# Aedelon/MASt3R-SLAM

Measured on AMD Instinct MI355X. Metric: keyframe-pairs/sec (512x512 two-view infer+match+GN), higher is better.
Workload: dtype fp16

## Files before the change

### mast3r-slam_amd/csrc/attention.hip

```cpp
#include "gemm_common.h"
#include <cstdlib>
#include <type_traits>

namespace {

using m3gemm::bf16x8;
using m3gemm::f32x4;
using m3gemm::bf16_t;
using m3gemm::glds16;
using m3gemm::pack16;
using m3gemm::mfma16;
using m3gemm::DT_BF16;
using m3gemm::DT_F16;
typedef __attribute__((ext_vector_type(4))) short bf16x4;
typedef float f32x2 __attribute__((ext_vector_type(2)));

constexpr int kThreads = 256;
constexpr int QROWS = 128;
constexpr int KT = 64;
constexpr int HD = 64;
constexpr int kTileBytes = KT * HD * 2;
constexpr int kLds = 4 * kTileBytes;

using m3gemm::pack_bf16;

struct AttnArgs {
    const bf16_t *Q, *K, *V;
    bf16_t *O;
    int q_row_stride, kv_row_stride, o_row_stride;
    long long q_batch_stride, kv_batch_stride, o_batch_stride;
    int Tq, Tk, heads, nbatch, kv_batch_shift;
    float scale_log2e;
};

#ifndef M3_ATTN_ABL
#define M3_ATTN_ABL 0
#endif
#ifndef M3_ATTN_EXP
#define M3_ATTN_EXP 0
#endif
constexpr float kDefer = 8.0f;
template <int QT, int DT, int MODE, int PVDT = DT>
__global__ void __launch_bounds__(kThreads, (MODE == 1 && QT == 2) ? 3 : 4)
k_attn(const AttnArgs a) {
    static_assert(MODE != 2 || PVDT == DT_BF16, "the deferred-maximum loop needs the fp32 exponent range of bf16 for P");
    constexpr int QR = QT * 64;
    __shared__ __attribute__((aligned(16))) unsigned char lds[kLds];
    const int tid = threadIdx.x, lane = tid & 63, wave = tid >> 6;
    const int lq = lane & 15, g = lane >> 4;
    const int nq = (a.Tq + QR - 1) / QR, nwg = gridDim.x;
    const int per = nwg >> 3, rem = nwg & 7, xcd = blockIdx.x & 7;
    const int id = (xcd < rem ? xcd * (per + 1) : rem * (per + 1) + (xcd - rem) * per) + (blockIdx.x >> 3);
    const int qblk = id % nq, head = (id / nq) % a.heads, b = id / (nq * a.heads);
    const int kvb = (b + a.kv_batch_shift) % a.nbatch;
    const bf16_t *Qp = a.Q + (size_t)b * a.q_batch_stride + head * HD;
    const bf16_t *Kp = a.K + (size_t)kvb * a.kv_batch_stride + head * HD;
    const bf16_t *Vp = a.V + (size_t)kvb * a.kv_batch_stride + head * HD;

    bf16x8 qf[QT][2];
#pragma unroll
    for (int qt = 0; qt < QT; ++qt) {
        int row = qblk * QR + wave * (16 * QT) + qt * 16 + lq;
        row = row < a.Tq ? row : a.Tq - 1;
#pragma unroll
        for (int ks = 0; ks < 2; ++ks)
            qf[qt][ks] = *reinterpret_cast<const bf16x8 *>(Qp + (size_t)row * a.q_row_stride + ks * 32 + g * 8);
    }

    const int srow = tid >> 3, sc = tid & 7;
    const int kch = sc ^ ((srow >> 1) & 7);
    const int vch = sc ^ (((srow >> 1) & 3) << 1);
    auto stage = [&](int t, int buf) {
        unsigned char *kb = lds + buf * 2 * kTileBytes, *vb = kb + kTileBytes;
#pragma unroll
        for (int i = 0; i < 2; ++i) {
            int kr = t * KT + i * 32 + srow;
            kr = kr < a.Tk ? kr : a.Tk - 1;
            const size_t row = (size_t)kr * a.kv_row_stride;
            glds16(Kp + row + kch * 8, kb + i * 4096 + wave * 1024);
            glds16(Vp + row + vch * 8, vb + i * 4096 + wave * 1024);
        }
    };

    f32x4 o[QT][4];
    float m_run[QT], l_run[QT];
    bool ovf = false;
    const int nt = (a.Tk + KT - 1) / KT;
    const int tq = lq >> 2, tp = lq & 3;

    auto run = [&](auto mode_tag) {
        constexpr int MD = decltype(mode_tag)::value;
        f32x4 l_acc[QT];
        bf16x8 ones;
#pragma unroll
        for (int j = 0; j < 8; ++j) ones[j] = (short)(PVDT == DT_BF16 ? 0x3F80 : 0x3C00);
#pragma unroll
        for (int qt = 0; qt < QT; ++qt) {
            m_run[qt] = -INFINITY; l_run[qt] = 0.f;
            l_acc[qt] = f32x4{0.f, 0.f, 0.f, 0.f};
#pragma unroll
            for (int dt = 0; dt < 4; ++dt) o[qt][dt] = f32x4{0.f, 0.f, 0.f, 0.f};
        }
        stage(0, 0);
        for (int t = 0; t < nt; ++t) {
            const int buf = t & 1;
            asm volatile("s_waitcnt vmcnt(0)" ::: "memory");
            m3gemm::lds_barrier();
            if (t + 1 < nt && !(M3_ATTN_ABL & 4)) stage(t + 1, buf ^ 1);
            const unsigned char *Ks = lds + ((M3_ATTN_ABL & 4) ? 0 : buf) * 2 * kTileBytes, *Vs = Ks + kTileBytes;

            if constexpr (MD == 2) {
                bool big = false;
#pragma unroll
                for (int qt = 0; qt < QT; ++qt) big |= l_acc[qt][0] > 0x1p60f;
                if (t > 0 && __any(big)) {
                    asm volatile("; rare path" ::: "memory");
#pragma unroll
                    for (int qt = 0; qt < QT; ++qt) {
                        const bool hit = l_acc[qt][0] > 0x1p60f;
                        ovf |= !(l_acc[qt][0] <= 0x1p100f);
                        const float alpha = hit ? 0x1p-64f : 1.0f;
                        m_run[qt] += hit ? 64.0f : 0.0f;
#pragma unroll
                        for (int r = 0; r < 4; ++r) l_acc[qt][r] *= alpha;
#pragma unroll
                        for (int dt = 0; dt < 4; ++dt)
#pragma unroll
                            for (int r = 0; r < 4; ++r) o[qt][dt][r] *= alpha;
                    }
                }
            }

            f32x4 s[QT][4];
#pragma unroll
            for (int qt = 0; qt < QT; ++qt) {
                const float c0 = (MD >= 1 && t > 0) ? -m_run[qt] : 0.f;
#pragma unroll
                for (int kt = 0; kt < 4; ++kt) s[qt][kt] = f32x4{c0, c0, c0, c0};
            }
#pragma unroll
            for (int ks = 0; ks < 2; ++ks)
#pragma unroll
                for (int kt = 0; kt < 4; ++kt) {
                    const int r = kt * 16 + lq;
                    const int c = (ks * 4 + g) ^ ((r >> 1) & 7);
                    bf16x8 kf;
                    if ((M3_ATTN_ABL & 1) && t > 0) { kf = qf[0][ks]; asm volatile("" : "+v"(kf)); }
                    else kf = *reinterpret_cast<const bf16x8 *>(Ks + r * 128 + c * 16);
#pragma unroll
                    for (int qt = 0; qt < QT; ++qt)
                        s[qt][kt] = mfma16<DT>(kf, qf[qt][ks], s[qt][kt]);
                }

            if (t == nt - 1 && (a.Tk & (KT - 1))) {
                const int kbase = t * KT + g * 4;
#pragma unroll
                for (int qt = 0; qt < QT; ++qt)
#pragma unroll
                    for (int kt = 0; kt < 4; ++kt)
#pragma unroll
                        for (int r = 0; r < 4; ++r)
                            if (kbase + kt * 16 + r >= a.Tk) s[qt][kt][r] = -INFINITY;
            }

            bf16x8 pf[QT][2];
            auto tile_max = [&](int qt) {
                float mx = fmaxf(__builtin_fmaxf(s[qt][0][0], s[qt][0][1]), s[qt][0][2]);
#pragma unroll
                for (int kt = 0; kt < 4; ++kt)
#pragma unroll
                    for (int r = (kt == 0 ? 3 : 0); r < 4; r += 2)
                        mx = (r + 1 < 4) ? fmaxf(__builtin_fmaxf(mx, s[qt][kt][r]), s[qt][kt][r + 1]) : fmaxf(mx, s[qt][kt][r]);
                mx = fmaxf(mx, __shfl_xor(mx, 16, 64));
                return fmaxf(mx, __shfl_xor(mx, 32, 64));
            };
            auto pack_p = [&](int qt) {
#pragma unroll
                for (int kk = 0; kk < 2; ++kk) {
                    union { unsigned u[4]; bf16x8 v; } pk;
                    pk.u[0] = pack16<PVDT>(s[qt][2 * kk][0], s[qt][2 * kk][1]);
                    pk.u[1] = pack16<PVDT>(s[qt][2 * kk][2], s[qt][2 * kk][3]);
                    pk.u[2] = pack16<PVDT>(s[qt][2 * kk + 1][0], s[qt][2 * kk + 1][1]);
                    pk.u[3] = pack16<PVDT>(s[qt][2 * kk + 1][2], s[qt][2 * kk + 1][3]);
                    pf[qt][kk] = pk.v;
                }
            };
            if constexpr (MD == 2) {
#pragma unroll
                for (int qt = 0; qt < QT; ++qt) {
                    if (t == 0) {
                        const float mx = tile_max(qt);
                        m_run[qt] = mx;
#pragma unroll
                        for (int kt = 0; kt < 4; ++kt)
#pragma unroll
                            for (int r = 0; r < 4; ++r) s[qt][kt][r] -= mx;
                    }
#pragma unroll
                    for (int kt = 0; kt < 4; ++kt)
#pragma unroll
                        for (int r = 0; r < 4; ++r) s[qt][kt][r] = (M3_ATTN_EXP >= 4) ? s[qt][kt][r] : __builtin_amdgcn_exp2f(s[qt][kt][r]);
#if M3_ATTN_EXP == 1
                    for (int kt = 0; kt < 4; ++kt) for (int r = 0; r < 4; ++r) l_run[qt] += s[qt][kt][r];
#endif
#if M3_ATTN_EXP == 5
                    pf[qt][0] = ones; pf[qt][1] = ones;
                    asm volatile("" :: "v"(s[qt][0]), "v"(s[qt][1]), "v"(s[qt][2]), "v"(s[qt][3]));
#else
                    pack_p(qt);
#endif
                }
            } else if constexpr (MD == 1) {
#pragma unroll
                for (int qt = 0; qt < QT; ++qt) {
                    const float mx = tile_max(qt);
                    if (t == 0) {
                        m_run[qt] = mx;
#pragma unroll
                        for (int kt = 0; kt < 4; ++kt)
#pragma unroll
                            for (int r = 0; r < 4; ++r) s[qt][kt][r] -= mx;
                    } else if (__any(mx > kDefer)) {
                        asm volatile("; rare path: keep it a branch (if-converted, its 32 subtracts + selects ran on every tile)" ::: "memory");
                        const float delta = fmaxf(mx, 0.f);
                        const float alpha = __builtin_amdgcn_exp2f(-delta);
                        m_run[qt] += delta;
                        l_run[qt] *= alpha;
#pragma unroll
                        for (int dt = 0; dt < 4; ++dt)
#pragma unroll
                            for (int r = 0; r < 4; ++r) o[qt][dt][r] *= alpha;
#pragma unroll
                        for (int kt = 0; kt < 4; ++kt)
#pragma unroll
                            for (int r = 0; r < 4; ++r) s[qt][kt][r] -= delta;
                    }
                    f32x2 rs2 = {0.f, 0.f};
#pragma unroll
                    for (int kt = 0; kt < 4; ++kt) {
#pragma unroll
                        for (int r = 0; r < 4; ++r) s[qt][kt][r] = __builtin_amdgcn_exp2f(s[qt][kt][r]);
                        rs2 += f32x2{s[qt][kt][0], s[qt][kt][1]};
                        rs2 += f32x2{s[qt][kt][2], s[qt][kt][3]};
                    }
                    l_run[qt] += rs2.x + rs2.y;
                    pack_p(qt);
                }
            } else {
#pragma unroll
                for (int qt = 0; qt < QT; ++qt) {
                    float mx = s[qt][0][0];
#pragma unroll
                    for (int kt = 0; kt < 4; ++kt)
#pragma unroll
                        for (int r = 0; r < 4; ++r) mx = fmaxf(mx, s[qt][kt][r]);
                    mx = fmaxf(mx, __shfl_xor(mx, 16, 64));
                    mx = fmaxf(mx, __shfl_xor(mx, 32, 64));
                    const float m_new = fmaxf(m_run[qt], mx);
                    const float alpha = __builtin_amdgcn_exp2f((m_run[qt] - m_new) * a.scale_log2e);
                    const float mb = m_new * a.scale_log2e;
                    m_run[qt] = m_new;
                    float rs = 0.f;
#pragma unroll
                    for (int kt = 0; kt < 4; ++kt)
#pragma unroll
                        for (int r = 0; r < 4; ++r) {
                            const float p = __builtin_amdgcn_exp2f(s[qt][kt][r] * a.scale_log2e - mb);
                            s[qt][kt][r] = p;
                            rs += p;
                        }
                    l_run[qt] = l_run[qt] * alpha + rs;
                    if (!__all(alpha == 1.0f)) {
#pragma unroll
                        for (int dt = 0; dt < 4; ++dt)
#pragma unroll
                            for (int r = 0; r < 4; ++r) o[qt][dt][r] *= alpha;
                    }
                    pack_p(qt);
                }
            }

#pragma unroll
            for (int kk = 0; kk < 2; ++kk) {
#pragma unroll
                for (int dt = 0; dt < 4; ++dt) {
                    union { bf16x4 h[2]; bf16x8 v; } vf;
                    if ((M3_ATTN_ABL & 2) && t > 0) { vf.v = qf[0][kk]; asm volatile("" : "+v"(vf.v)); }
                    else
#pragma unroll
                    for (int half = 0; half < 2; ++half) {
                        const int row = (2 * kk + half) * 16 + g * 4 + tq;
                        const int ch = (dt * 2 + (tp >> 1)) ^ (((row >> 1) & 3) << 1);
                        const unsigned char *p = Vs + row * 128 + ch * 16 + (tp & 1) * 8;
                        vf.h[half] = __builtin_amdgcn_ds_read_tr16_b64_v4i16(
                            (__attribute__((address_space(3))) bf16x4 *)p);
                    }
#pragma unroll
                    for (int qt = 0; qt < QT; ++qt)
                        o[qt][dt] = mfma16<PVDT>(vf.v, pf[qt][kk], o[qt][dt]);
                }
                if constexpr (MD == 2) {
#pragma unroll
                    for (int qt = 0; qt < QT; ++qt) l_acc[qt] = mfma16<PVDT>(ones, pf[qt][kk], l_acc[qt]);
                }
            }
        }
        m3gemm::lds_barrier();
        if constexpr (MD == 2 && M3_ATTN_EXP != 1) {
#pragma unroll
            for (int qt = 0; qt < QT; ++qt) l_run[qt] = l_acc[qt][0];
        } else {
#pragma unroll
            for (int qt = 0; qt < QT; ++qt) {
                float l = l_run[qt];
                l += __shfl_xor(l, 16, 64);
                l_run[qt] = l + __shfl_xor(l, 32, 64);
            }
        }
    };

    if constexpr (MODE == 2) {
        run(std::integral_constant<int, 2>{});
        bool bad = ovf;
#pragma unroll
        for (int qt = 0; qt < QT; ++qt) {
            bad |= !(l_run[qt] > 0.f && l_run[qt] <= 0x1p100f);
            float osum = 0.f;
#pragma unroll
            for (int dt = 0; dt < 4; ++dt) osum += (o[qt][dt][0] + o[qt][dt][1]) + (o[qt][dt][2] + o[qt][dt][3]);
            bad |= !(fabsf(osum) < INFINITY);
        }
#if M3_ATTN_EXP == 3
        bad = true;
#endif
        int *flag = reinterpret_cast<int *>(lds);
        if (tid == 0) *flag = 0;
        m3gemm::lds_barrier();
        if (__any(bad) && lane == 0) atomicOr(flag, 1);
        m3gemm::lds_barrier();
        const int redo = *reinterpret_cast<volatile int *>(flag);
        m3gemm::lds_barrier();
        if (redo) run(std::integral_constant<int, 1>{});
    } else {
        run(std::integral_constant<int, MODE>{});
    }

#pragma unroll
    for (int qt = 0; qt < QT; ++qt) {
        const float inv = 1.0f / l_run[qt];
        const int row = qblk * QR + wave * (16 * QT) + qt * 16 + lq;
        if (row >= a.Tq) continue;
        bf16_t *op = a.O + (size_t)b * a.o_batch_stride + (size_t)row * a.o_row_stride + head * HD;
#pragma unroll
        for (int dt = 0; dt < 4; ++dt) {
            uint2 w;
            w.x = pack16<DT>(o[qt][dt][0] * inv, o[qt][dt][1] * inv);
            w.y = pack16<DT>(o[qt][dt][2] * inv, o[qt][dt][3] * inv);
            *reinterpret_cast<uint2 *>(op + dt * 16 + g * 4) = w;
        }
    }
}

template <int DT>
__global__ void __launch_bounds__(kThreads)
k_rope2d(bf16_t *__restrict__ X, const int *__restrict__ pos_yx, const float *__restrict__ cs, int row_stride,
         int tokens, int heads, int tokens_per_image) {
    const int idx = blockIdx.x * kThreads + threadIdx.x;
    const int total = tokens * heads * 2;
    if (idx >= total) return;
    const int blk = idx & 1, head = (idx >> 1) % heads, tok = (idx >> 1) / heads;
    const int pos = pos_yx[(tok % tokens_per_image) * 2 + blk];
    bf16_t *p = X + (size_t)tok * row_stride + head * HD + blk * 32;
    union { uint4 q[4]; bf16_t h[32]; } v;
#pragma unroll
    for (int i = 0; i < 4; ++i) v.q[i] = reinterpret_cast<const uint4 *>(p)[i];
    const float *t = cs + (size_t)pos * 32;
#pragma unroll
    for (int i = 0; i < 16; ++i) {
        const float c = t[2 * i], sn = t[2 * i + 1];
        const float x1 = m3gemm::lo16<DT>(v.h[i]), x2 = m3gemm::lo16<DT>(v.h[i + 16]);
        const unsigned pk = pack16<DT>(x1 * c - x2 * sn, x2 * c + x1 * sn);
        v.h[i] = (bf16_t)(pk & 0xffff);
        v.h[i + 16] = (bf16_t)(pk >> 16);
    }
#pragma unroll
    for (int i = 0; i < 4; ++i) reinterpret_cast<uint4 *>(p)[i] = v.q[i];
}

}

extern "C" {

static int attention_launch(const void *Q, const void *K, const void *V, void *O, int q_row_stride, int kv_row_stride,
                            int o_row_stride, int64_t q_batch_stride, int64_t kv_batch_stride, int64_t o_batch_stride,
                            int nbatch, int heads, int Tq, int Tk, int kv_batch_shift, float scale, int dtype, bool pre,
                            void *stream) {
    M3_REQUIRE(Q && K && V && O && nbatch > 0 && heads > 0 && Tq > 0 && Tk > 0);
    M3_REQUIRE((dtype == DT_BF16 || dtype == DT_F16 || (dtype == 2 && pre)) && ((int64_t)Tq / 64 + 1) * heads * nbatch < (1ll << 31));
    M3_REQUIRE(q_row_stride % 8 == 0 && kv_row_stride % 8 == 0 && o_row_stride % 4 == 0);
    M3_REQUIRE(kv_batch_shift >= 0);
    AttnArgs a;
    a.Q = (const bf16_t *)Q; a.K = (const bf16_t *)K; a.V = (const bf16_t *)V; a.O = (bf16_t *)O;
    a.q_row_stride = q_row_stride; a.kv_row_stride = kv_row_stride; a.o_row_stride = o_row_stride;
    a.q_batch_stride = q_batch_stride; a.kv_batch_stride = kv_batch_stride; a.o_batch_stride = o_batch_stride;
    a.Tq = Tq; a.Tk = Tk; a.heads = heads; a.nbatch = nbatch; a.kv_batch_shift = kv_batch_shift;
    a.scale_log2e = scale * 1.4426950408889634f;
    const int64_t wg128 = (int64_t)m3_cdiv(Tq, QROWS) * heads * nbatch;
    const int64_t wg64 = (int64_t)m3_cdiv(Tq, 64) * heads * nbatch;
    hipStream_t st = (hipStream_t)stream;
    static const bool safe_bf16 = [] { const char *e = getenv("M3_ATTN_SAFE"); return e && atoi(e) != 0; }();
#define M3_ATTN(QTV, GRID)                                                                                  \
    do {                                                                                                    \
        if (dtype == 2) hipLaunchKernelGGL((k_attn<QTV, DT_F16, 2, DT_BF16>), dim3((unsigned)(GRID)), dim3(kThreads), 0, st, a); \
        else if (dtype == DT_F16) { if (pre) hipLaunchKernelGGL((k_attn<QTV, DT_F16, 1>), dim3((unsigned)(GRID)), dim3(kThreads), 0, st, a); \
                               else hipLaunchKernelGGL((k_attn<QTV, DT_F16, 0>), dim3((unsigned)(GRID)), dim3(kThreads), 0, st, a); } \
        else { if (pre) { if (safe_bf16) hipLaunchKernelGGL((k_attn<QTV, DT_BF16, 1>), dim3((unsigned)(GRID)), dim3(kThreads), 0, st, a); \
                          else hipLaunchKernelGGL((k_attn<QTV, DT_BF16, 2>), dim3((unsigned)(GRID)), dim3(kThreads), 0, st, a); }          \
               else hipLaunchKernelGGL((k_attn<QTV, DT_BF16, 0>), dim3((unsigned)(GRID)), dim3(kThreads), 0, st, a); }                    \
    } while (0)
    if (wg128 >= 512) M3_ATTN(2, wg128); else M3_ATTN(1, wg64);
#undef M3_ATTN
    M3_CHECK_LAUNCH("m3_attention");
    return M3_OK;
}

int m3_attention_dt(const void *Q, const void *K, const void *V, void *O, int q_row_stride, int kv_row_stride,
                    int o_row_stride, int64_t q_batch_stride, int64_t kv_batch_stride, int64_t o_batch_stride,
                    int nbatch, int heads, int Tq, int Tk, int kv_batch_shift, float scale, int dtype, void *stream) {
    return attention_launch(Q, K, V, O, q_row_stride, kv_row_stride, o_row_stride, q_batch_stride, kv_batch_stride,
                            o_batch_stride, nbatch, heads, Tq, Tk, kv_batch_shift, scale, dtype, false, stream);
}
int m3_attention_prescaled_dt(const void *Q, const void *K, const void *V, void *O, int q_row_stride, int kv_row_stride,
                              int o_row_stride, int64_t q_batch_stride, int64_t kv_batch_stride, int64_t o_batch_stride,
                              int nbatch, int heads, int Tq, int Tk, int kv_batch_shift, int dtype, void *stream) {
    return attention_launch(Q, K, V, O, q_row_stride, kv_row_stride, o_row_stride, q_batch_stride, kv_batch_stride,
                            o_batch_stride, nbatch, heads, Tq, Tk, kv_batch_shift, 1.0f, dtype, true, stream);
}
int m3_rope2d_dt(void *X, const int32_t *pos_yx, const float *cos_sin, int row_stride, int tokens, int heads,
                 int tokens_per_image, int dtype, void *stream) {
    M3_REQUIRE(X && pos_yx && cos_sin && tokens > 0 && heads > 0 && tokens_per_image > 0 && row_stride % 8 == 0);
    M3_REQUIRE(dtype == DT_BF16 || dtype == DT_F16);
    const int64_t total = (int64_t)tokens * heads * 2;
    if (dtype == DT_F16)
        hipLaunchKernelGGL(k_rope2d<DT_F16>, dim3(m3_cdiv(total, kThreads)), dim3(kThreads), 0, (hipStream_t)stream,
                           (bf16_t *)X, pos_yx, cos_sin, row_stride, tokens, heads, tokens_per_image);
    else
        hipLaunchKernelGGL(k_rope2d<DT_BF16>, dim3(m3_cdiv(total, kThreads)), dim3(kThreads), 0, (hipStream_t)stream,
                           (bf16_t *)X, pos_yx, cos_sin, row_stride, tokens, heads, tokens_per_image);
    M3_CHECK_LAUNCH("m3_rope2d");
    return M3_OK;
}

}
```

### mast3r-slam_amd/csrc/gemm_common.h

```cpp
#pragma once
#include "common.h"
#include "../../include/m3slam_model.h"

namespace m3gemm {

typedef __attribute__((ext_vector_type(8))) short bf16x8;
typedef __attribute__((ext_vector_type(4))) float f32x4;
typedef unsigned short bf16_t;

constexpr int BK = 64;

__device__ __forceinline__ float bf2f(bf16_t v) { return __uint_as_float((unsigned)v << 16); }
__device__ __forceinline__ bf16_t f2bf(float f) {
    unsigned u = __float_as_uint(f);
    if ((u & 0x7fffffffu) > 0x7f800000u) return (bf16_t)((u >> 16) | 0x40);
    return (bf16_t)((u + 0x7fffu + ((u >> 16) & 1u)) >> 16);
}
typedef float f32x2 __attribute__((ext_vector_type(2)));
__device__ __forceinline__ f32x2 gelu_erf2(f32x2 x) {
    f32x2 z = x * 0.70710678118654752f;
    z.x = __builtin_amdgcn_fmed3f(z.x, -3.0f, 3.0f);
    z.y = __builtin_amdgcn_fmed3f(z.y, -3.0f, 3.0f);
    const f32x2 u = z * z;
    f32x2 p = (f32x2)(4.074053805e-08f);
    p = __builtin_elementwise_fma(p, u, (f32x2)(-1.944763426e-06f));
    p = __builtin_elementwise_fma(p, u, (f32x2)(4.105960033e-05f));
    p = __builtin_elementwise_fma(p, u, (f32x2)(-5.110292695e-04f));
    p = __builtin_elementwise_fma(p, u, (f32x2)(4.235391971e-03f));
    p = __builtin_elementwise_fma(p, u, (f32x2)(-2.510276809e-02f));
    p = __builtin_elementwise_fma(p, u, (f32x2)(1.110792086e-01f));
    p = __builtin_elementwise_fma(p, u, (f32x2)(-3.753148019e-01f));
    p = __builtin_elementwise_fma(p, u, (f32x2)(1.128268361e+00f));
    const f32x2 hx = x * 0.5f;
    return __builtin_elementwise_fma(hx, z * p, hx);
}

typedef __bf16 m3_bf16x2 __attribute__((ext_vector_type(2)));
typedef _Float16 m3_f16x2 __attribute__((ext_vector_type(2)));
__device__ __forceinline__ unsigned pack_bf16(float lo, float hi) {
    return __builtin_bit_cast(unsigned, __builtin_convertvector(f32x2{lo, hi}, m3_bf16x2));
}

enum { DT_BF16 = 0, DT_F16 = 1 };
typedef __attribute__((ext_vector_type(8))) _Float16 f16x8;
template <int DT> __device__ __forceinline__ unsigned pack16(float lo, float hi) {
    if constexpr (DT == DT_BF16) return pack_bf16(lo, hi);
    else return __builtin_bit_cast(unsigned, __builtin_convertvector(f32x2{lo, hi}, m3_f16x2));
}
template <int DT> __device__ __forceinline__ float lo16(unsigned q) {
    if constexpr (DT == DT_BF16) return __uint_as_float(q << 16);
    else return (float)__builtin_bit_cast(_Float16, (unsigned short)(q & 0xffffu));
}
template <int DT> __device__ __forceinline__ float hi16(unsigned q) {
    if constexpr (DT == DT_BF16) return __uint_as_float(q & 0xffff0000u);
    else return (float)__builtin_bit_cast(_Float16, (unsigned short)(q >> 16));
}
template <int DT> __device__ __forceinline__ f32x4 mfma16(bf16x8 a, bf16x8 b, f32x4 c) {
    if constexpr (DT == DT_BF16) return __builtin_amdgcn_mfma_f32_16x16x32_bf16(a, b, c, 0, 0, 0);
    else return __builtin_amdgcn_mfma_f32_16x16x32_f16(__builtin_bit_cast(f16x8, a), __builtin_bit_cast(f16x8, b), c, 0, 0, 0);
}

typedef __attribute__((ext_vector_type(8))) short s16x8;
__device__ __forceinline__ bf16x8 relu_frag(bf16x8 v) {
    return __builtin_elementwise_max(v, (bf16x8)(short)0);
}

__device__ __forceinline__ void glds16(const void *g, void *lds_wave_base) {
    __builtin_amdgcn_global_load_lds((const __attribute__((address_space(1))) unsigned *)g,
                                     (__attribute__((address_space(3))) unsigned *)lds_wave_base, 16, 0, 0);
}

__device__ __forceinline__ void lds_barrier() {
    __builtin_amdgcn_sched_barrier(0);
    asm volatile("s_waitcnt lgkmcnt(0)" ::: "memory");
    __builtin_amdgcn_s_barrier();
    __builtin_amdgcn_sched_barrier(0);
}

struct GemmArgs {
    const bf16_t *A;
    const bf16_t *W;
    const float *bias;
    void *C;
    const void *R;
    const bf16_t *zero16;
    int M, N, K, ldc;
    int H, Wd, Cin, OH, OW, stride;
    const int *rope_pos;
    float rope_log2_base;
    int tokens_per_image, rope_cols;
    int ln_gsz, ln_tops;
    int rope_pmax;
    int q_cols;
    float q_scale;
    const bf16_t *W2;
    const float *bias2;
    long long a_gstride, c_gstride;
    int groups;
    int splits;
    int slices;
    float *C2;
    int dt;
    int relu_a;
    int v_bf16;
    void *C16;
    float *stats_out;
    int stats_w;
    const void *R_lo;
    void *C_lo;
    const float *ln_stats;
    const float *ln_colsum, *ln_colsum2;
    int ln_slots;
    float ln_eps;
    long long ln_gstride, stats_gstride;
};

template <int EPI>
__device__ __forceinline__ GemmArgs select_group(const GemmArgs &in, int grp) {
    GemmArgs g = in;
    if (grp == 1) {
        constexpr long long esz = (EPI == 2  || EPI == 3 ) ? 4 : 2;
        g.A = in.A + in.a_gstride;
        g.W = in.W2;
        g.bias = in.bias2;
        g.C = reinterpret_cast<unsigned char *>(in.C) + in.c_gstride * esz;
        if (in.R) g.R = reinterpret_cast<const unsigned char *>(in.R) + in.c_gstride * esz;
        if (in.C16) g.C16 = reinterpret_cast<unsigned char *>(in.C16) + in.c_gstride * 2;
        if (in.C_lo) {
            g.C_lo = reinterpret_cast<unsigned char *>(in.C_lo) + in.c_gstride * 2;
            if (in.R) g.R = reinterpret_cast<const unsigned char *>(in.R) + in.c_gstride * 2;
            if (in.R_lo) g.R_lo = reinterpret_cast<const unsigned char *>(in.R_lo) + in.c_gstride * 2;
        }
        if (in.stats_out) g.stats_out = in.stats_out + in.stats_gstride;
        if (in.ln_stats) { g.ln_stats = in.ln_stats + in.ln_gstride; g.ln_colsum = in.ln_colsum2; }
    }
    return g;
}

enum { EPI_BF16 = 0, EPI_BF16_GELU = 1, EPI_F32 = 2, EPI_F32_ACCUM = 3, EPI_BF16_RELU = 4, EPI_BF16_ADD = 5,
       EPI_BF16_ROPE = 6,
       EPI_RELU_HEAD4 = 7  };


template <int EPI, int DT = DT_BF16>
__device__ __forceinline__ void store_tile(const GemmArgs &g, f32x4 v, int m, int n) {
    if (m >= g.M || n >= g.N) return;
    if (EPI != EPI_BF16_ROPE && g.bias) {
        const float4 b = *reinterpret_cast<const float4 *>(g.bias + n);
        v[0] += b.x; v[1] += b.y; v[2] += b.z; v[3] += b.w;
    }
    const size_t off = (size_t)m * g.ldc + n;
    if (EPI == EPI_F32 || EPI == EPI_F32_ACCUM) {
        float *C = reinterpret_cast<float *>(g.C) + off;
        if (EPI == EPI_F32_ACCUM) {
            const float4 r = *reinterpret_cast<const float4 *>(reinterpret_cast<const float *>(g.R) + off);
            v[0] += r.x; v[1] += r.y; v[2] += r.z; v[3] += r.w;
        }
        *reinterpret_cast<float4 *>(C) = make_float4(v[0], v[1], v[2], v[3]);
    } else {
        if (EPI == EPI_BF16_GELU) {
            const f32x2 lo = gelu_erf2(f32x2{v[0], v[1]}), hi = gelu_erf2(f32x2{v[2], v[3]});
            v[0] = lo.x; v[1] = lo.y; v[2] = hi.x; v[3] = hi.y;
        }
        if (EPI == EPI_BF16_ADD) {
            const uint2 r = *reinterpret_cast<const uint2 *>(reinterpret_cast<const bf16_t *>(g.R) + off);
            v[0] += lo16<DT>(r.x); v[1] += hi16<DT>(r.x); v[2] += lo16<DT>(r.y); v[3] += hi16<DT>(r.y);
        }
        if (EPI == EPI_BF16_RELU) {
#pragma unroll
            for (int e = 0; e < 4; ++e) v[e] = v[e] > 0.f ? v[e] : 0.f;
        }
        uint2 o;
        if (EPI == EPI_BF16_ROPE && DT == DT_F16 && g.v_bf16 && n >= g.rope_cols) {
            o.x = pack16<DT_BF16>(v[0], v[1]); o.y = pack16<DT_BF16>(v[2], v[3]);
        } else {
            o.x = pack16<DT>(v[0], v[1]); o.y = pack16<DT>(v[2], v[3]);
        }
        *reinterpret_cast<uint2 *>(reinterpret_cast<bf16_t *>(g.C) + off) = o;
    }
}

struct RopeCoef { float4 c, s; };
struct RopeFreq { float rev[4]; };
__device__ __forceinline__ RopeFreq rope_freqs(const GemmArgs &g, int lane) {
    RopeFreq f;
    const int fi = (lane >> 4) * 4;
#pragma unroll
    for (int k = 0; k < 4; ++k) f.rev[k] = exp2f(-(float)(fi + k) * (g.rope_log2_base * (1.0f / 16.0f))) * 0.15915494309189535f;
    return f;
}
constexpr int kRopeTableRows = 64;
__device__ __forceinline__ void rope_table_build(const GemmArgs &g, float *tab, int tid, int nthreads) {
    for (int e = tid; e < g.rope_pmax * 16; e += nthreads) {
        const int p = e >> 4, f = e & 15;
        const float rev = exp2f(-(float)f * (g.rope_log2_base * (1.0f / 16.0f))) * 0.15915494309189535f;
        const float ang = (float)p * rev;
        tab[p * 32 + f] = __builtin_amdgcn_cosf(ang);
        tab[p * 32 + 16 + f] = __builtin_amdgcn_sinf(ang);
    }
}
__device__ __forceinline__ int2 rope_pos_of(const GemmArgs &g, int m) {
    const int mm = m < g.M ? m : g.M - 1;
    return *reinterpret_cast<const int2 *>(g.rope_pos + (size_t)(mm % g.tokens_per_image) * 2);
}
template <int NJ>
__device__ __forceinline__ void rope_load(const GemmArgs &g, RopeCoef (&cf)[NJ / 2], int n_base, int lane, const RopeFreq &fr,
                                          int2 pyx, const float *ropet = nullptr) {
    const int fi = (lane >> 4) * 4;
#pragma unroll
    for (int blk = 0; blk < NJ / 2; ++blk) {
        if (n_base + 32 * blk >= g.rope_cols) continue;
        const int axis = ((n_base + 32 * blk) >> 5) & 1;
        if (ropet) {
            int p = axis ? pyx.y : pyx.x;
            p = p < g.rope_pmax ? p : g.rope_pmax - 1;
            p = p > 0 ? p : 0;
            const float *row = ropet + p * 32 + fi;
            cf[blk].c = *reinterpret_cast<const float4 *>(row);
            cf[blk].s = *reinterpret_cast<const float4 *>(row + 16);
        } else {
            const float pos = (float)(axis ? pyx.y : pyx.x);
            cf[blk].c = make_float4(__builtin_amdgcn_cosf(pos * fr.rev[0]), __builtin_amdgcn_cosf(pos * fr.rev[1]),
                                    __builtin_amdgcn_cosf(pos * fr.rev[2]), __builtin_amdgcn_cosf(pos * fr.rev[3]));
            cf[blk].s = make_float4(__builtin_amdgcn_sinf(pos * fr.rev[0]), __builtin_amdgcn_sinf(pos * fr.rev[1]),
                                    __builtin_amdgcn_sinf(pos * fr.rev[2]), __builtin_amdgcn_sinf(pos * fr.rev[3]));
        }
    }
}
template <int NJ>
__device__ __forceinline__ void rope_apply(const GemmArgs &g, f32x4 *t, const RopeCoef (&cf)[NJ / 2], const float4 *bj,
                                           int n_base) {
#pragma unroll
    for (int blk = 0; blk < NJ / 2; ++blk) {
        f32x4 &a = t[2 * blk], &b = t[2 * blk + 1];
        const float4 ba = bj[2 * blk], bb = bj[2 * blk + 1];
        const f32x2 a0 = f32x2{a[0], a[1]} + f32x2{ba.x, ba.y}, a1 = f32x2{a[2], a[3]} + f32x2{ba.z, ba.w};
        const f32x2 b0 = f32x2{b[0], b[1]} + f32x2{bb.x, bb.y}, b1 = f32x2{b[2], b[3]} + f32x2{bb.z, bb.w};
        if (n_base + 32 * blk >= g.rope_cols) {
            a = f32x4{a0.x, a0.y, a1.x, a1.y}; b = f32x4{b0.x, b0.y, b1.x, b1.y};
            continue;
        }
        const f32x2 c0 = {cf[blk].c.x, cf[blk].c.y}, c1 = {cf[blk].c.z, cf[blk].c.w};
        const f32x2 s0 = {cf[blk].s.x, cf[blk].s.y}, s1 = {cf[blk].s.z, cf[blk].s.w};
        f32x2 ra0 = __builtin_elementwise_fma(a0, c0, -(b0 * s0)), ra1 = __builtin_elementwise_fma(a1, c1, -(b1 * s1));
        f32x2 rb0 = __builtin_elementwise_fma(b0, c0, a0 * s0), rb1 = __builtin_elementwise_fma(b1, c1, a1 * s1);
        if (n_base + 32 * blk < g.q_cols) {
            const f32x2 qs = {g.q_scale, g.q_scale};
            ra0 = ra0 * qs; ra1 = ra1 * qs; rb0 = rb0 * qs; rb1 = rb1 * qs;
        }
        a = f32x4{ra0.x, ra0.y, ra1.x, ra1.y}; b = f32x4{rb0.x, rb0.y, rb1.x, rb1.y};
    }
}
template <int NJ>
__device__ __forceinline__ void rope_strip(const GemmArgs &g, f32x4 *t, int m, int n_base, int lane) {
    if (m >= g.M) return;
    const int fi = (lane >> 4) * 4;
    float4 bj[NJ];
#pragma unroll
    for (int j = 0; j < NJ; ++j)
        bj[j] = (g.bias && n_base + j * 16 + fi < g.N) ? *reinterpret_cast<const float4 *>(g.bias + n_base + j * 16 + fi)
                                                       : make_float4(0.f, 0.f, 0.f, 0.f);
    RopeCoef cf[NJ / 2];
    rope_load<NJ>(g, cf, n_base, lane, rope_freqs(g, lane), g.rope_pos ? rope_pos_of(g, m) : int2{0, 0});
    rope_apply<NJ>(g, t, cf, bj, n_base);
}

__device__ __forceinline__ float dpp_sum8(float v) {
    v += __builtin_bit_cast(float, __builtin_amdgcn_update_dpp(0, __builtin_bit_cast(int, v), 0xB1, 0xF, 0xF, true));
    v += __builtin_bit_cast(float, __builtin_amdgcn_update_dpp(0, __builtin_bit_cast(int, v), 0x4E, 0xF, 0xF, true));
    v += __builtin_bit_cast(float, __builtin_amdgcn_update_dpp(0, __builtin_bit_cast(int, v), 0x141, 0xF, 0xF, true));
    return v;
}
__device__ __forceinline__ unsigned dpp_xor1(unsigned v) {
    return (unsigned)__builtin_amdgcn_update_dpp(0, (int)v, 0xB1, 0xF, 0xF, true);
}

__device__ __forceinline__ float ln_tree8(const float (&x)[8]) {
    return ((x[0] + x[1]) + (x[2] + x[3])) + ((x[4] + x[5]) + (x[6] + x[7]));
}
struct LnLoads { float4 v[4]; };
__device__ __forceinline__ float2 ln_mean_rstd(float s, float q, int cols, float eps) {
    const float inv = 1.0f / (float)cols;
    const float mean = s * inv;
    const float var = fmaxf(__builtin_fmaf(-mean, mean, q * inv), 0.f);
    return make_float2(mean, rsqrtf(var + eps));
}
template <int ROWS>
__device__ __forceinline__ LnLoads ln_row_issue(const GemmArgs &g, int m0, int tid) {
    LnLoads L;
    const int pair = (tid < 2 * ROWS ? tid : 0) >> 2, q = tid & 3;
    const int node = q < g.ln_tops ? q : g.ln_tops - 1;
    int m = m0 + 2 * pair;
    m = m < g.M - 1 ? m : g.M - 2;
    const float4 *p = reinterpret_cast<const float4 *>(g.ln_stats + ((size_t)node * g.ln_gsz * g.M + m) * 2);
    const size_t slot_stride = (size_t)g.M / 2;
#pragma unroll
    for (int i = 0; i < 4; ++i) L.v[i] = p[(size_t)(i < g.ln_gsz ? i : g.ln_gsz - 1) * slot_stride];
    return L;
}
template <int ROWS>
__device__ __forceinline__ float4 ln_row_finish(const GemmArgs &g, const LnLoads &L, int m0, int tid) {
    const bool live = (tid & 3) < g.ln_tops;
    float4 u[4];
#pragma unroll
    for (int i = 0; i < 4; ++i) {
        const bool on = live && i < g.ln_gsz;
        u[i] = make_float4(on ? L.v[i].x : 0.f, on ? L.v[i].y : 0.f, on ? L.v[i].z : 0.f, on ? L.v[i].w : 0.f);
    }
    const float node[4] = {(u[0].x + u[1].x) + (u[2].x + u[3].x), (u[0].y + u[1].y) + (u[2].y + u[3].y),
                           (u[0].z + u[1].z) + (u[2].z + u[3].z), (u[0].w + u[1].w) + (u[2].w + u[3].w)};
    float t[4];
#pragma unroll
    for (int k = 0; k < 4; ++k) {
        const int b = __builtin_bit_cast(int, node[k]);
        const float t0 = __builtin_bit_cast(float, __builtin_amdgcn_update_dpp(0, b, 0x00, 0xF, 0xF, true));
        const float t1 = __builtin_bit_cast(float, __builtin_amdgcn_update_dpp(0, b, 0x55, 0xF, 0xF, true));
        const float t2 = __builtin_bit_cast(float, __builtin_amdgcn_update_dpp(0, b, 0xAA, 0xF, 0xF, true));
        const float t3 = __builtin_bit_cast(float, __builtin_amdgcn_update_dpp(0, b, 0xFF, 0xF, 0xF, true));
        t[k] = ((t0 + t1) + t2) + t3;
    }
    const float2 a = ln_mean_rstd(t[0], t[1], g.K, g.ln_eps), b2 = ln_mean_rstd(t[2], t[3], g.K, g.ln_eps);
    return make_float4(a.x, a.y, b2.x, b2.y);
}
template <int ROWS>
__device__ __forceinline__ float4 ln_row_stats(const GemmArgs &g, int m0, int tid) {
    return ln_row_finish<ROWS>(g, ln_row_issue<ROWS>(g, m0, tid), m0, tid);
}
template <int NJ> constexpr int stats_stage_offset() { return (16 * ((NJ == 4) ? 256 : NJ * 64 + 16) + 15) & ~15; }
template <int TROWS, int NI, int NJ, int WN>
__device__ __forceinline__ void stats_tile_finalize(const GemmArgs &g, const unsigned char *lds, int wave_stride, int wst_off,
                                                    int m0, int n0, int tid) {
    constexpr int WROWS = 16 * NI, LPW = NJ / 2, LEAVES = WN * LPW;
    if (tid >= TROWS) return;
    const int wr = tid / WROWS, rr = tid - wr * WROWS;
    const int lpu = g.stats_w >> 5;
    const int m = m0 + tid;
    for (int k = 0; k * lpu < LEAVES; ++k) {
        float s[8], q[8];
#pragma unroll
        for (int i = 0; i < 8; ++i) {
            const bool on = i < lpu;
            const int l = k * lpu + (on ? i : 0);
            const int wc = l / LPW, sl = l - wc * LPW;
            const float2 v = *reinterpret_cast<const float2 *>(lds + (wr * WN + wc) * wave_stride + wst_off + (sl * WROWS + rr) * 8);
            s[i] = on ? v.x : 0.f; q[i] = on ? v.y : 0.f;
        }
        const int n = n0 + k * g.stats_w;
        if (m < g.M && n < g.N)
            *reinterpret_cast<float2 *>(g.stats_out + ((size_t)(n / g.stats_w) * g.M + m) * 2) = make_float2(ln_tree8(s), ln_tree8(q));
    }
}
template <int ROWS>
__device__ __forceinline__ void ln_table_store(float2 *tab, const float4 &mr, int tid) {
    if (tid < 2 * ROWS && (tid & 3) == 0) {
        tab[2 * (tid >> 2)] = make_float2(mr.x, mr.y);
        tab[2 * (tid >> 2) + 1] = make_float2(mr.z, mr.w);
    }
}
template <int ROWS>
__device__ __forceinline__ void ln_row_table(const GemmArgs &g, float2 *tab, int m0, int tid) {
    ln_table_store<ROWS>(tab, ln_row_stats<ROWS>(g, m0, tid), tid);
}

template <int EPI, int NI, int NJ = 4, int DT = DT_BF16, int TPMAX = 4, bool RESID_AHEAD = true, bool ALIGNED = false>
__device__ __forceinline__ void epilogue_rows(const GemmArgs &g, f32x4 (&acc)[NI][NJ], unsigned char *wlds,
                                              int m_base, int n_base, int lane, const float2 *lnt = nullptr, int lrow = 0,
                                              const float *ropet = nullptr) {
    constexpr bool F32OUT = (EPI == EPI_F32 || EPI == EPI_F32_ACCUM);
    constexpr bool F32LDS = F32OUT || EPI == EPI_BF16_ADD;
    const int r = lane & 15, gq = lane >> 4;
    const bool aligned = ((reinterpret_cast<size_t>(g.C) & 15) == 0) && (g.ldc % (F32OUT ? 4 : 8) == 0) &&
                         (F32OUT || g.N % 8 == 0) &&
                         (!(EPI == EPI_F32_ACCUM || EPI == EPI_BF16_ADD) || (reinterpret_cast<size_t>(g.R) & 15) == 0);
    if (!ALIGNED && !aligned) {
#pragma unroll
        for (int i = 0; i < NI; ++i) {
            if (EPI == EPI_BF16_ROPE) rope_strip<NJ>(g, acc[i], m_base + i * 16 + r, n_base, lane);
#pragma unroll
            for (int j = 0; j < NJ; ++j) store_tile<EPI, DT>(g, acc[i][j], m_base + i * 16 + r, n_base + j * 16 + gq * 4);
        }
        return;
    }
    float4 bj[NJ];
    if (g.bias) {
#pragma unroll
        for (int j = 0; j < NJ; ++j) {
            const int n = n_base + j * 16 + gq * 4;
            bj[j] = *reinterpret_cast<const float4 *>(g.bias + (n < g.N ? n : g.N - 4));
        }
#pragma unroll
        for (int j = 0; j < NJ; ++j)
            if (n_base + j * 16 + gq * 4 >= g.N) bj[j] = make_float4(0.f, 0.f, 0.f, 0.f);
    } else {
#pragma unroll
        for (int j = 0; j < NJ; ++j) bj[j] = make_float4(0.f, 0.f, 0.f, 0.f);
    }
    if (F32LDS) {
        constexpr bool SWZ32 = F32OUT && (NJ == 4);
        constexpr int RS = SWZ32 ? 256 : NJ * 64 + 16;
        constexpr bool RESID = (EPI == EPI_F32_ACCUM || EPI == EPI_BF16_ADD);
        constexpr int PT = 1;
        constexpr int PR = 16 * PT;
        constexpr int CPR = F32OUT ? NJ * 4 : NJ * 2;
        constexpr int NIT = PR * CPR / 64;
        static_assert(!F32OUT || ((PR * RS + 15) & ~15) == stats_stage_offset<NJ>(), "stats_tile_finalize reads the staging where the epilogue wrote it");
        float2 *wst = reinterpret_cast<float2 *>(wlds + ((PR * RS + 15) & ~15));
        uint4 q[RESID_AHEAD ? 2 : 1][RESID ? NIT : 1];
        auto load_resid = [&](int pass, uint4 (&dst)[RESID ? NIT : 1]) {
            if constexpr (RESID) {
                size_t off[NIT];
#pragma unroll
                for (int it = 0; it < NIT; ++it) {
                    const int c = it * 64 + lane, rl = c / CPR, ch = c - rl * CPR;
                    int m = m_base + pass * PR + rl, n = n_base + ch * (F32OUT ? 4 : 8);
                    m = m < g.M ? m : g.M - 1;
                    n = n < g.N ? n : 0;
                    off[it] = (size_t)m * g.ldc + n;
                }
                if (F32OUT && g.C_lo) {
#pragma unroll
                    for (int it = 0; it < NIT; ++it) {
                        const uint2 hi = *reinterpret_cast<const uint2 *>(reinterpret_cast<const bf16_t *>(g.R) + off[it]);
                        const uint2 lo = *reinterpret_cast<const uint2 *>(reinterpret_cast<const bf16_t *>(g.R_lo) + off[it]);
                        dst[it] = uint4{hi.x, hi.y, lo.x, lo.y};
                    }
                } else {
#pragma unroll
                    for (int it = 0; it < NIT; ++it)
                        dst[it] = F32OUT ? *reinterpret_cast<const uint4 *>(reinterpret_cast<const float *>(g.R) + off[it])
                                         : *reinterpret_cast<const uint4 *>(reinterpret_cast<const bf16_t *>(g.R) + off[it]);
                }
            }
        };
        if (RESID_AHEAD) load_resid(0, q[0]);
#pragma unroll
        for (int pass = 0; pass < NI / PT; ++pass) {
            if (RESID_AHEAD) { if (pass + 1 < NI / PT) load_resid(pass + 1, q[(pass + 1) & (RESID_AHEAD ? 1 : 0)]); }
            else load_resid(pass, q[0]);
#pragma unroll
            for (int ii = 0; ii < PT; ++ii)
#pragma unroll
                for (int j = 0; j < NJ; ++j) {
                    const f32x4 v = acc[pass * PT + ii][j];
                    *reinterpret_cast<float4 *>(wlds + (ii * 16 + r) * RS + ((SWZ32 ? ((j * 4 + gq) ^ (r & 7)) : (j * 4 + gq)) << 4)) =
                        make_float4(v[0] + bj[j].x, v[1] + bj[j].y, v[2] + bj[j].z, v[3] + bj[j].w);
                }
            asm volatile("s_waitcnt lgkmcnt(0)" ::: "memory");
            if (F32OUT) {
#pragma unroll
                for (int it = 0; it < NIT; ++it) {
                    const int c = it * 64 + lane, rl = c / CPR, ch = c - rl * CPR;
                    float4 v = *reinterpret_cast<const float4 *>(wlds + rl * RS + ((SWZ32 ? (ch ^ (rl & 7)) : ch) << 4));
                    const int m = m_base + pass * PR + rl, n = n_base + ch * 4;
                    if (EPI == EPI_F32_ACCUM) {
                        const uint4 u = q[RESID_AHEAD ? (pass & 1) : 0][it];
                        if (g.C_lo) {
                            v.x += lo16<DT>(u.x) + lo16<DT>(u.z); v.y += hi16<DT>(u.x) + hi16<DT>(u.z);
                            v.z += lo16<DT>(u.y) + lo16<DT>(u.w); v.w += hi16<DT>(u.y) + hi16<DT>(u.w);
                        } else {
                            v.x += __uint_as_float(u.x); v.y += __uint_as_float(u.y); v.z += __uint_as_float(u.z); v.w += __uint_as_float(u.w);
                        }
                    }
                    if (g.C_lo) {
                        const unsigned h0 = pack16<DT>(v.x, v.y), h1 = pack16<DT>(v.z, v.w);
                        const unsigned l0 = pack16<DT>(v.x - lo16<DT>(h0), v.y - hi16<DT>(h0));
                        const unsigned l1 = pack16<DT>(v.z - lo16<DT>(h1), v.w - hi16<DT>(h1));
                        const unsigned g0 = dpp_xor1(h0), g1 = dpp_xor1(h1), k0 = dpp_xor1(l0), k1 = dpp_xor1(l1);
                        if (!(lane & 1) && m < g.M && n < g.N) {
                            *reinterpret_cast<uint4 *>(reinterpret_cast<bf16_t *>(g.C16) + (size_t)m * g.ldc + n) = uint4{h0, h1, g0, g1};
                            *reinterpret_cast<uint4 *>(reinterpret_cast<bf16_t *>(g.C_lo) + (size_t)m * g.ldc + n) = uint4{l0, l1, k0, k1};
                        }
                    } else {
                    if (m < g.M && n < g.N)
                        *reinterpret_cast<float4 *>(reinterpret_cast<float *>(g.C) + (size_t)m * g.ldc + n) = v;
                    if (g.C16) {
                        const unsigned p0 = pack16<DT>(v.x, v.y), p1 = pack16<DT>(v.z, v.w);
                        const unsigned q0 = dpp_xor1(p0), q1 = dpp_xor1(p1);
                        if (!(lane & 1) && m < g.M && n < g.N)
                            *reinterpret_cast<uint4 *>(reinterpret_cast<bf16_t *>(g.C16) + (size_t)m * g.ldc + n) = uint4{p0, p1, q0, q1};
                    }
                    }
                    if (g.stats_out) {
                        const bool live = m < g.M && n < g.N;
                        const float s1 = dpp_sum8(live ? (v.x + v.y) + (v.z + v.w) : 0.f);
                        const float s2 = dpp_sum8(live ? (v.x * v.x + v.y * v.y) + (v.z * v.z + v.w * v.w) : 0.f);
                        if ((ch & 7) == 0)
                            wst[(ch >> 3) * (16 * NI) + pass * PR + rl] = make_float2(s1, s2);
                    }
                }
            } else {
#pragma unroll
                for (int it = 0; it < NIT; ++it) {
                    const int c = it * 64 + lane, rl = c / CPR, ch = c - rl * CPR;
                    const float4 a = *reinterpret_cast<const float4 *>(wlds + rl * RS + ch * 32);
                    const float4 b = *reinterpret_cast<const float4 *>(wlds + rl * RS + ch * 32 + 16);
                    const int m = m_base + pass * PR + rl, n = n_base + ch * 8;
                    const uint4 u = q[RESID_AHEAD ? (pass & 1) : 0][it];
                    uint4 o;
                    o.x = pack16<DT>(a.x + lo16<DT>(u.x), a.y + hi16<DT>(u.x));
                    o.y = pack16<DT>(a.z + lo16<DT>(u.y), a.w + hi16<DT>(u.y));
                    o.z = pack16<DT>(b.x + lo16<DT>(u.z), b.y + hi16<DT>(u.z));
                    o.w = pack16<DT>(b.z + lo16<DT>(u.w), b.w + hi16<DT>(u.w));
                    if (m < g.M && n < g.N)
                        *reinterpret_cast<uint4 *>(reinterpret_cast<bf16_t *>(g.C) + (size_t)m * g.ldc + n) = o;
                }
            }
            asm volatile("" ::: "memory");
        }
    } else {
        constexpr bool SWZ = (NJ == 4);
        constexpr int RS = SWZ ? 128 : NJ * 32 + 16;
        constexpr int TP = NI < TPMAX ? NI : TPMAX;
        constexpr int PR = 16 * TP, CPR = NJ * 2;
        RopeFreq fr{};
        if constexpr (EPI == EPI_BF16_ROPE) { if (g.rope_pos && !ropet) fr = rope_freqs(g, lane); }
        if (lnt) {
            float4 csj[NJ];
#pragma unroll
            for (int j = 0; j < NJ; ++j) {
                const int n = n_base + j * 16 + gq * 4;
                csj[j] = *reinterpret_cast<const float4 *>(g.ln_colsum + (n < g.N ? n : g.N - 4));
            }
#pragma unroll
            for (int i = 0; i < NI; ++i) {
                const float2 mr = lnt[lrow + i * 16 + r];
#pragma unroll
                for (int j = 0; j < NJ; ++j) {
                    f32x4 &v = acc[i][j];
                    v[0] = mr.y * (v[0] - mr.x * csj[j].x); v[1] = mr.y * (v[1] - mr.x * csj[j].y);
                    v[2] = mr.y * (v[2] - mr.x * csj[j].z); v[3] = mr.y * (v[3] - mr.x * csj[j].w);
                }
            }
        }
#pragma unroll
        for (int pass = 0; pass < NI / TP; ++pass) {
            RopeCoef cf[EPI == EPI_BF16_ROPE ? TP : 1][NJ / 2];
            if constexpr (EPI == EPI_BF16_ROPE) {
                int2 pyx[TP];
#pragma unroll
                for (int ii = 0; ii < TP; ++ii) pyx[ii] = int2{0, 0};
                if (g.rope_pos) {
#pragma unroll
                    for (int ii = 0; ii < TP; ++ii) pyx[ii] = rope_pos_of(g, m_base + (pass * TP + ii) * 16 + r);
                }
#pragma unroll
                for (int ii = 0; ii < TP; ++ii) rope_load<NJ>(g, cf[ii], n_base, lane, fr, pyx[ii], ropet);
            }
#pragma unroll
            for (int ii = 0; ii < TP; ++ii) {
                const int i = pass * TP + ii;
                if constexpr (EPI == EPI_BF16_ROPE) rope_apply<NJ>(g, acc[i], cf[ii], bj, n_base);
#pragma unroll
                for (int j = 0; j < NJ; ++j) {
                    f32x4 v = acc[i][j];
                    if constexpr (EPI != EPI_BF16_ROPE) { v[0] += bj[j].x; v[1] += bj[j].y; v[2] += bj[j].z; v[3] += bj[j].w; }
                    if (EPI == EPI_BF16_GELU) {
                        const f32x2 lo = gelu_erf2(f32x2{v[0], v[1]}), hi = gelu_erf2(f32x2{v[2], v[3]});
                        v[0] = lo.x; v[1] = lo.y; v[2] = hi.x; v[3] = hi.y;
                    }
                    if (EPI == EPI_BF16_RELU) {
#pragma unroll
                        for (int e = 0; e < 4; ++e) v[e] = v[e] > 0.f ? v[e] : 0.f;
                    }
                    uint2 pk;
                    if (EPI == EPI_BF16_ROPE && DT == DT_F16 && g.v_bf16 && n_base + (j >> 1) * 32 >= g.rope_cols) {
                        pk.x = pack16<DT_BF16>(v[0], v[1]); pk.y = pack16<DT_BF16>(v[2], v[3]);
                    } else {
                        pk.x = pack16<DT>(v[0], v[1]); pk.y = pack16<DT>(v[2], v[3]);
                    }
                    if constexpr (SWZ)
                        *reinterpret_cast<uint2 *>(wlds + (ii * 16 + r) * RS + (((j * 2 + (gq >> 1)) ^ ((r >> 1) & 7)) << 4) + (((gq ^ r) & 1) << 3)) = pk;
                    else
                        *reinterpret_cast<uint2 *>(wlds + (ii * 16 + r) * RS + (j * 16 + gq * 4) * 2) = pk;
                }
            }
            asm volatile("s_waitcnt lgkmcnt(0)" ::: "memory");
#pragma unroll
            for (int it = 0; it < PR * CPR / 64; ++it) {
                const int c = it * 64 + lane, rl = c / CPR, ch = c - rl * CPR;
                uint4 v = *reinterpret_cast<const uint4 *>(wlds + rl * RS + ((SWZ ? (ch ^ ((rl >> 1) & 7)) : ch) << 4));
                if (SWZ && (rl & 1)) v = uint4{v.z, v.w, v.x, v.y};
                const int m = m_base + pass * PR + rl, n = n_base + ch * 8;
                if (m < g.M && n < g.N)
                    *reinterpret_cast<uint4 *>(reinterpret_cast<bf16_t *>(g.C) + (size_t)m * g.ldc + n) = v;
            }
            asm volatile("" ::: "memory");
        }
    }
}

__device__ __forceinline__ size_t conv_k_offset(int kt, int Cin) {
    const int q = kt / 9, tap = kt - q * 9;
    return (size_t)tap * Cin + q * BK;
}

__device__ __forceinline__ int xcd_remap(int bid, int nwg) {
    const int q = nwg / 8, r = nwg % 8, xcd = bid % 8;
    return (xcd < r ? xcd * (q + 1) : r * (q + 1) + (xcd - r) * q) + bid / 8;
}

}
```

Baseline: 299.1.

## Stage K/V via buffer loads to LDS, peel first tile, precompute fragment offsets

Replaces global_load_lds staging of K/V tiles with raw buffer loads to LDS, using per-lane offsets and scalar wave offsets that are computed once. The clamped tail path is limited to the last partial tile. The first key tile is peeled into its own specialization, so the t==0 branches become compile-time. The running-max reference is kept as a vector register that seeds the QK accumulators directly. LDS fragment addresses for K and V reads are precomputed outside the loop, cutting per-iteration address arithmetic and VGPR pressure, at the cost of more code size and a new kv_row_stride limit.

```diff
diff --git a/mast3r-slam_amd/csrc/attention.hip b/mast3r-slam_amd/csrc/attention.hip
--- a/mast3r-slam_amd/csrc/attention.hip
+++ b/mast3r-slam_amd/csrc/attention.hip
@@ -7,7 +7,6 @@
 using m3gemm::bf16x8;
 using m3gemm::f32x4;
 using m3gemm::bf16_t;
-using m3gemm::glds16;
 using m3gemm::pack16;
 using m3gemm::mfma16;
 using m3gemm::DT_BF16;
@@ -40,6 +39,10 @@
 #define M3_ATTN_EXP 0
 #endif
 constexpr float kDefer = 8.0f;
+__device__ __forceinline__ float mul_then_sub(float a, float b, float c) {
+#pragma clang fp contract(off)
+    return a * b - c;
+}
 template <int QT, int DT, int MODE, int PVDT = DT>
 __global__ void __launch_bounds__(kThreads, (MODE == 1 && QT == 2) ? 3 : 4)
 k_attn(const AttnArgs a) {
@@ -70,23 +73,47 @@
     const int srow = tid >> 3, sc = tid & 7;
     const int kch = sc ^ ((srow >> 1) & 7);
     const int vch = sc ^ (((srow >> 1) & 3) << 1);
-    auto stage = [&](int t, int buf) {
-        unsigned char *kb = lds + buf * 2 * kTileBytes, *vb = kb + kTileBytes;
-#pragma unroll
-        for (int i = 0; i < 2; ++i) {
-            int kr = t * KT + i * 32 + srow;
-            kr = kr < a.Tk ? kr : a.Tk - 1;
-            const size_t row = (size_t)kr * a.kv_row_stride;
-            glds16(Kp + row + kch * 8, kb + i * 4096 + wave * 1024);
-            glds16(Vp + row + vch * 8, vb + i * 4096 + wave * 1024);
+    const int nt = (a.Tk + KT - 1) / KT;
+    const unsigned row_bytes = (unsigned)a.kv_row_stride * 2u;
+    const unsigned k_lane = (unsigned)srow * row_bytes + kch * 16, v_lane = (unsigned)srow * row_bytes + vch * 16;
+    unsigned char *const lds_wave = lds + __builtin_amdgcn_readfirstlane(wave) * 1024;
+    auto stage = [&](int t, int stage_off) {
+        unsigned char *kb = lds_wave + stage_off, *vb = kb + kTileBytes;
+        const auto kr = m3gemm::stream_rsrc(Kp + (size_t)t * KT * a.kv_row_stride);
+        const auto vr = m3gemm::stream_rsrc(Vp + (size_t)t * KT * a.kv_row_stride);
+        if (t == nt - 1 && (a.Tk & (KT - 1))) {
+            asm volatile("; key tail: rows past Tk are staged from the last row" ::: "memory");
+            const int last = a.Tk - 1 - t * KT;
+            int sr = tid >> 3;
+            asm volatile("" : "+v"(sr));
+#pragma unroll
+            for (int i = 0; i < 2; ++i) {
+                const int r = i * 32 + sr;
+                const unsigned row = (unsigned)(r < last ? r : last) * row_bytes;
+                m3gemm::blds16(kr, row + kch * 16, 0, kb + i * 4096);
+                m3gemm::blds16(vr, row + vch * 16, 0, vb + i * 4096);
+            }
+        } else {
+#pragma unroll
+            for (int i = 0; i < 2; ++i) {
+                m3gemm::blds16(kr, k_lane, i * 32 * row_bytes, kb + i * 4096);
+                m3gemm::blds16(vr, v_lane, i * 32 * row_bytes, vb + i * 4096);
+            }
         }
     };
 
     f32x4 o[QT][4];
     float m_run[QT], l_run[QT];
     bool ovf = false;
-    const int nt = (a.Tk + KT - 1) / KT;
     const int tq = lq >> 2, tp = lq & 3;
+    int k_frag[2], v_frag[4];
+#pragma unroll
+    for (int ks = 0; ks < 2; ++ks) k_frag[ks] = lq * 128 + ((ks * 4 + g) ^ (lq >> 1)) * 16;
+#pragma unroll
+    for (int dt = 0; dt < 4; ++dt) {
+        const int row = g * 4 + tq;
+        v_frag[dt] = row * 128 + ((dt * 2 + (tp >> 1)) ^ (((row >> 1) & 3) << 1)) * 16 + (tp & 1) * 8;
+    }
 
     auto run = [&](auto mode_tag) {
         constexpr int MD = decltype(mode_tag)::value;
@@ -101,26 +128,35 @@
 #pragma unroll
             for (int dt = 0; dt < 4; ++dt) o[qt][dt] = f32x4{0.f, 0.f, 0.f, 0.f};
         }
-        stage(0, 0);
-        for (int t = 0; t < nt; ++t) {
-            const int buf = t & 1;
+        f32x4 c0v[QT];
+#pragma unroll
+        for (int qt = 0; qt < QT; ++qt) c0v[qt] = f32x4{0.f, 0.f, 0.f, 0.f};
+        auto reference = [&](int qt) { return -c0v[qt][0]; };
+        auto new_reference = [&](int qt, float m_ref) {
+            const float c0 = -m_ref;
+            c0v[qt] = f32x4{c0, c0, c0, c0};
+        };
+        constexpr int kStage = 2 * kTileBytes;
+        auto tile = [&](const int t, auto first_c) {
+            constexpr bool FIRST = decltype(first_c)::value;
+            const int flip = (M3_ATTN_ABL & 4) ? 0 : (t & 1) * kStage;
             asm volatile("s_waitcnt vmcnt(0)" ::: "memory");
             m3gemm::lds_barrier();
-            if (t + 1 < nt && !(M3_ATTN_ABL & 4)) stage(t + 1, buf ^ 1);
-            const unsigned char *Ks = lds + ((M3_ATTN_ABL & 4) ? 0 : buf) * 2 * kTileBytes, *Vs = Ks + kTileBytes;
-
-            if constexpr (MD == 2) {
+            if (t + 1 < nt && !(M3_ATTN_ABL & 4)) stage(t + 1, flip ^ kStage);
+            const unsigned char *Ks = lds + flip, *Vs = Ks + kTileBytes;
+
+            if constexpr (MD == 2 && !FIRST) {
                 bool big = false;
 #pragma unroll
                 for (int qt = 0; qt < QT; ++qt) big |= l_acc[qt][0] > 0x1p60f;
-                if (t > 0 && __any(big)) {
+                if (__any(big)) {
                     asm volatile("; rare path" ::: "memory");
 #pragma unroll
                     for (int qt = 0; qt < QT; ++qt) {
                         const bool hit = l_acc[qt][0] > 0x1p60f;
                         ovf |= !(l_acc[qt][0] <= 0x1p100f);
                         const float alpha = hit ? 0x1p-64f : 1.0f;
-                        m_run[qt] += hit ? 64.0f : 0.0f;
+                        new_reference(qt, reference(qt) + (hit ? 64.0f : 0.0f));
 #pragma unroll
                         for (int r = 0; r < 4; ++r) l_acc[qt][r] *= alpha;
 #pragma unroll
@@ -132,21 +168,21 @@
             }
 
             f32x4 s[QT][4];
-#pragma unroll
-            for (int qt = 0; qt < QT; ++qt) {
-                const float c0 = (MD >= 1 && t > 0) ? -m_run[qt] : 0.f;
-#pragma unroll
-                for (int kt = 0; kt < 4; ++kt) s[qt][kt] = f32x4{c0, c0, c0, c0};
-            }
+            if constexpr (MD >= 1 && !FIRST) {
+#pragma unroll
+                for (int qt = 0; qt < QT; ++qt) asm("" : "+v"(c0v[qt]));
+            }
+#pragma unroll
+            for (int qt = 0; qt < QT; ++qt)
+#pragma unroll
+                for (int kt = 0; kt < 4; ++kt) s[qt][kt] = c0v[qt];
 #pragma unroll
             for (int ks = 0; ks < 2; ++ks)
 #pragma unroll
                 for (int kt = 0; kt < 4; ++kt) {
-                    const int r = kt * 16 + lq;
-                    const int c = (ks * 4 + g) ^ ((r >> 1) & 7);
                     bf16x8 kf;
-                    if ((M3_ATTN_ABL & 1) && t > 0) { kf = qf[0][ks]; asm volatile("" : "+v"(kf)); }
-                    else kf = *reinterpret_cast<const bf16x8 *>(Ks + r * 128 + c * 16);
+                    if ((M3_ATTN_ABL & 1) && !FIRST && t > 0) { kf = qf[0][ks]; asm volatile("" : "+v"(kf)); }
+                    else kf = *reinterpret_cast<const bf16x8 *>(Ks + kt * 2048 + k_frag[ks]);
 #pragma unroll
                     for (int qt = 0; qt < QT; ++qt)
                         s[qt][kt] = mfma16<DT>(kf, qf[qt][ks], s[qt][kt]);
@@ -188,9 +224,9 @@
             if constexpr (MD == 2) {
 #pragma unroll
                 for (int qt = 0; qt < QT; ++qt) {
-                    if (t == 0) {
+                    if constexpr (FIRST) {
                         const float mx = tile_max(qt);
-                        m_run[qt] = mx;
+                        new_reference(qt, mx);
 #pragma unroll
                         for (int kt = 0; kt < 4; ++kt)
 #pragma unroll
@@ -214,8 +250,8 @@
 #pragma unroll
                 for (int qt = 0; qt < QT; ++qt) {
                     const float mx = tile_max(qt);
-                    if (t == 0) {
-                        m_run[qt] = mx;
+                    if (FIRST) {
+                        new_reference(qt, mx);
 #pragma unroll
                         for (int kt = 0; kt < 4; ++kt)
 #pragma unroll
@@ -224,7 +260,7 @@
                         asm volatile("; rare path: keep it a branch (if-converted, its 32 subtracts + selects ran on every tile)" ::: "memory");
                         const float delta = fmaxf(mx, 0.f);
                         const float alpha = __builtin_amdgcn_exp2f(-delta);
-                        m_run[qt] += delta;
+                        new_reference(qt, reference(qt) + delta);
                         l_run[qt] *= alpha;
 #pragma unroll
                         for (int dt = 0; dt < 4; ++dt)
@@ -265,7 +301,9 @@
                     for (int kt = 0; kt < 4; ++kt)
 #pragma unroll
                         for (int r = 0; r < 4; ++r) {
-                            const float p = __builtin_amdgcn_exp2f(s[qt][kt][r] * a.scale_log2e - mb);
+                            const float e = (kt == 3 && r == 3) ? mul_then_sub(s[qt][kt][r], a.scale_log2e, mb)
+                                                                : __builtin_fmaf(s[qt][kt][r], a.scale_log2e, -mb);
+                            const float p = __builtin_amdgcn_exp2f(e);
                             s[qt][kt][r] = p;
                             rs += p;
                         }
@@ -285,13 +323,11 @@
 #pragma unroll
                 for (int dt = 0; dt < 4; ++dt) {
                     union { bf16x4 h[2]; bf16x8 v; } vf;
-                    if ((M3_ATTN_ABL & 2) && t > 0) { vf.v = qf[0][kk]; asm volatile("" : "+v"(vf.v)); }
+                    if ((M3_ATTN_ABL & 2) && !FIRST && t > 0) { vf.v = qf[0][kk]; asm volatile("" : "+v"(vf.v)); }
                     else
 #pragma unroll
                     for (int half = 0; half < 2; ++half) {
-                        const int row = (2 * kk + half) * 16 + g * 4 + tq;
-                        const int ch = (dt * 2 + (tp >> 1)) ^ (((row >> 1) & 3) << 1);
-                        const unsigned char *p = Vs + row * 128 + ch * 16 + (tp & 1) * 8;
+                        const unsigned char *p = Vs + (2 * kk + half) * 2048 + v_frag[dt];
                         vf.h[half] = __builtin_amdgcn_ds_read_tr16_b64_v4i16(
                             (__attribute__((address_space(3))) bf16x4 *)p);
                     }
@@ -304,7 +340,10 @@
                     for (int qt = 0; qt < QT; ++qt) l_acc[qt] = mfma16<PVDT>(ones, pf[qt][kk], l_acc[qt]);
                 }
             }
-        }
+        };
+        stage(0, 0);
+        if constexpr (MD >= 1) tile(0, std::true_type{});
+        for (int t = (MD >= 1 ? 1 : 0); t < nt; ++t) tile(t, std::false_type{});
         m3gemm::lds_barrier();
         if constexpr (MD == 2 && M3_ATTN_EXP != 1) {
 #pragma unroll
@@ -398,6 +437,7 @@
     M3_REQUIRE(Q && K && V && O && nbatch > 0 && heads > 0 && Tq > 0 && Tk > 0);
     M3_REQUIRE((dtype == DT_BF16 || dtype == DT_F16 || (dtype == 2 && pre)) && ((int64_t)Tq / 64 + 1) * heads * nbatch < (1ll << 31));
     M3_REQUIRE(q_row_stride % 8 == 0 && kv_row_stride % 8 == 0 && o_row_stride % 4 == 0);
+    M3_REQUIRE(kv_row_stride >= 0 && kv_row_stride < (1 << 23));
     M3_REQUIRE(kv_batch_shift >= 0);
     AttnArgs a;
     a.Q = (const bf16_t *)Q; a.K = (const bf16_t *)K; a.V = (const bf16_t *)V; a.O = (bf16_t *)O;
diff --git a/mast3r-slam_amd/csrc/gemm_common.h b/mast3r-slam_amd/csrc/gemm_common.h
--- a/mast3r-slam_amd/csrc/gemm_common.h
+++ b/mast3r-slam_amd/csrc/gemm_common.h
@@ -68,6 +68,12 @@
 __device__ __forceinline__ void glds16(const void *g, void *lds_wave_base) {
     __builtin_amdgcn_global_load_lds((const __attribute__((address_space(1))) unsigned *)g,
                                      (__attribute__((address_space(3))) unsigned *)lds_wave_base, 16, 0, 0);
+}
+__device__ __forceinline__ __amdgpu_buffer_rsrc_t stream_rsrc(const void *base) {
+    return __builtin_amdgcn_make_buffer_rsrc(const_cast<void *>(base), 0, 0x7ffffff0, 0x00020000);
+}
+__device__ __forceinline__ void blds16(__amdgpu_buffer_rsrc_t r, unsigned lane_off, unsigned wave_off, void *lds_wave_base) {
+    __builtin_amdgcn_raw_ptr_buffer_load_lds(r, (__attribute__((address_space(3))) void *)lds_wave_base, 16, lane_off, wave_off, 0, 0);
 }
 
 __device__ __forceinline__ void lds_barrier() {
```

After: 303.4, median of 6. +1.4%, better.
